# acerbilab/pyvbmc

Measured on AMD Instinct MI355X. Metric: ELBO+entropy evals/sec at D=10, K=50, N=400, Ns=1e6 (1e6-sample-equivalent evals/s), higher is better.
Workload: dtype f64; 1 GPU; BASELINE config 3 per GPU: D=10 K=50 N=400 S=1, Ns=1000000 MC samples per GPU (job Ns=1000000), value+grad _neg_elcbo with soft bounds, eps=philox; parallelism=single GPU

## Files before the change

pyvbmc_amd/_lib.py:

```python
import ctypes as C
import os
import sys
import threading
from pathlib import Path

import numpy as np

_HERE = Path(__file__).resolve().parent
LIB_PATH = Path(os.environ.get("VBMC_HIP_LIB", _HERE / "libvbmc_hip.so"))

EPS_RESIDENT, EPS_PHILOX = 0, 1
MEAN_ZERO, MEAN_CONST, MEAN_NEGQUAD = 0, 1, 2
E_ARG, E_HIP, E_RCCL, E_NODEV, E_UNSUP, E_NONFINITE = -1, -2, -3, -4, -5, -6
W_GP_CHANGED = 1
W_NOT_FUSED = 2


class VbmcHipError(RuntimeError):
    def __init__(self, code, msg):
        super().__init__(f"libvbmc_hip error {code}: {msg}")
        self.code = code


class NoDeviceError(VbmcHipError):
# ... 274 lines not shown
        return bool(b.value), n.value

    def synchronize(self):
        self.check(self._lib.vbmc_synchronize(self._h))

    def set_timing(self, on):
        self.check(self._lib.vbmc_set_timing(self._h, int(on) if on else 0))

    def set_option(self, key, value):
        self.check(self._lib.vbmc_set_option(self._h, key.encode(), int(value)))

    def last_entmc_plan(self):
        out = (C.c_int * 4)()
        self.check(self._lib.vbmc_last_entmc_plan(self._h, out))
        return {"kernel": ("valu", "ws", "small", "mfma", "adam_fused", "ws", "ws")[out[0]] if out[0] >= 0 else None, "rg": out[1],
                "chunks": out[2], "resident_draws": bool(out[3]), "span": out[0] in (5, 6), "adam_tail": out[0] == 6}

    def philox_normals(self, K, n_half, D, seed, row_begin=0, row_count=None):
        row_count = n_half - row_begin if row_count is None else row_count
        out = np.empty((K, row_count, D))
        self.check(self._lib.vbmc_philox_normals(self._h, K, n_half, D, C.c_uint64(seed), row_begin, row_count, ptr(out)))
        return out

    def armed_stats(self):
        out = (C.c_uint64 * 6)()
        self.check(self._lib.vbmc_armed_stats(self._h, out))
        return dict(zip(("hits", "cancels", "late", "ident_checked", "ident_bad", "lost"), (int(v) for v in out)))

    def last_elbo_raw(self, D, K):
        out = np.empty(1 + D * K + 2 * K + D)
        self.check(self._lib.vbmc_last_elbo_raw(self._h, ptr(out), out.size))
# ... 126 lines not shown
```

pyvbmc_amd/csrc/api_elbo.hip:

```cpp
#include <algorithm>
#include <chrono>
#include <cstdlib>
#include <cmath>
#include <cstring>

#include "common.h"
#include "entropy_args.h"

static double soft_bound_loss(const std::vector<double>& x, const double* lb, const double* ub,
                              double tol_con, std::vector<double>* dy) {
  double y = 0.0;
  if (dy) dy->assign(x.size(), 0.0);
  for (size_t i = 0; i < x.size(); ++i) {
    if (x[i] >= lb[i] && x[i] <= ub[i]) continue;
    const double ell = (ub[i] - lb[i]) * tol_con;
    if (x[i] < lb[i]) {
      const double t = (lb[i] - x[i]) / ell;
      y += 0.5 * t * t;
      if (dy) (*dy)[i] = (x[i] - lb[i]) / (ell * ell);
    }
    if (x[i] > ub[i]) {
      const double t = (x[i] - ub[i]) / ell;
      y += 0.5 * t * t;
      if (dy) (*dy)[i] = (x[i] - ub[i]) / (ell * ell);
// ... 208 lines not shown
    if (spin) {
      ctl = ctl_word(ctx, seq_out);
      *(volatile uint64_t*)ctl = 0;
      __builtin_ia32_sfence();
      pa.go = ctl;
      pa.go_seq = seq_out;
      pa.go_timeout = (uint64_t)(ARM_DEVICE_WAIT_MS * 1e5);
      pa.dead = ctx->hd_done + 5;
      plan.a.cancel = ctl;
    }
    HSTAMP(1);
    rc2 = launch_prep(ctx, pa);
    if (rc2) return rc2;
    polled_out = false;
    if (mc) {
      rc2 = entmc_launch_main(ctx, plan);
      if (rc2) return rc2;
      GenSlice ahead_gen;
      DoneSignal done;
      if (can_poll) {
        if (ahead_ok) ahead_gen = entmc_ahead_slice(ctx, plan);
        done.cnt = ctx->d_done_cnt;
        done.sub = ctx->d_done_sub;
        {
          static const int sub_min = [] { const char* e = getenv("VBMC_FIN_SUB_MIN"); return e ? atoi(e) : 256; }();
          done.sub_min = sub_min;
        }
        done.flag = ctx->hd_done;
        done.seq = seq_out;
        done.host_out = raw_out;
        done.host_n = n_raw;
        done.cancel = ctl;
        if (ident) {
          done.ident_src = (const uint64_t*)(ctx->d_done_cnt + 12);
          done.ident_dst = ctx->hd_done + 1;
          done.ident_seed = seed;
        }
        polled_out = true;
        ident_out_flag = ident;
      }
      const GenSlice* gen_here = ahead_gen.n_blocks > 0 ? &ahead_gen : nullptr;
      if (!multi) {
        rc2 = entmc_launch_finish(ctx, plan, polled_out ? stage + n_res : raw_out, gen_here, polled_out ? &done : nullptr);
        if (rc2) return rc2;
      } else {
        rc2 = entmc_launch_finish(ctx, plan, raw_out, nullptr, nullptr);
        if (rc2) return rc2;
        rc2 = comm_allreduce_sum(ctx, raw_out, n_raw);
        if (rc2) return rc2;
        if (polled_out) {
          done.host_out = raw_host;
          rc2 = entmc_launch_publish(ctx, raw_out, done, gen_here);
          if (rc2) return rc2;
        } else {
          HIP_TRY(ctx, hipMemcpyAsync(ctx->h_pinned + n_res, raw_out, sizeof(double) * n_raw,
                                      hipMemcpyDeviceToHost, ctx->stream));
        }
// ... 23 lines not shown
      sp.armed = false;
      const bool force_late = ctx->opt_arm_late_test > 0 && --ctx->opt_arm_late_test == 0;
      if (!force_late && std::chrono::duration<double, std::milli>(clk::now() - sp.t_armed).count() < sp.limit_ms + ARM_LATE_SLACK_MS) {
        ++sp.hits;
        used_armed = true;
        polled = true;
        cur_seq = sp.seq;
        check_ident = sp.ident;
        HSTAMP(1);
      } else {
        *(volatile uint64_t*)ctl_word(ctx, sp.seq) = ~(uint64_t)0;
        __builtin_ia32_sfence();
        HIP_TRY(ctx, stream_wait(ctx));
        HIP_TRY(ctx, hipMemsetAsync(ctx->d_done_cnt, 0, sizeof(int) * 16, ctx->stream));
        HIP_TRY(ctx, hipMemsetAsync(ctx->d_done_sub, 0, sizeof(int) * 16 * 64, ctx->stream));
        ctx->gen_cur = sp.gen_cur_before;
        ctx->ahead.valid = sp.ahead_before_valid;
        ctx->ahead.seed = sp.ahead_before_seed;
        ctx->ahead.buf = sp.ahead_before_buf;
        ctx->ahead.frac = sp.ahead_before_frac;
        ++sp.cancels;
        ++sp.late;
      }
    } else {
      spec_disarm(ctx);
    }
  }
  if (!used_armed) {
    rc = issue(opts->seed, false, polled, cur_seq);
    if (rc) return rc;
// ... 136 lines not shown
    const volatile uint64_t* dead = ctx->h_done + 5;
    unsigned spins = 0;
    for (;;) {
      if (*f == want) break;
      if (*dead == want) return 1;
      __builtin_ia32_pause();
      if ((++spins & 0xFFFF) == 0 && us_since(t_wait) > 5e6) return 2;
    }
    __atomic_thread_fence(__ATOMIC_ACQUIRE);
    return 0;
  };
  auto redo_unarmed = [&](const char* why) -> int {
    HIP_TRY(ctx, stream_wait(ctx));
    HIP_TRY(ctx, hipMemsetAsync(ctx->d_done_cnt, 0, sizeof(int) * 16, ctx->stream));
        HIP_TRY(ctx, hipMemsetAsync(ctx->d_done_sub, 0, sizeof(int) * 16 * 64, ctx->stream));
    ctx->ahead.valid = false;
    if (ctx->ident_retry) return vbmc_fail(ctx, VBMC_E_HIP, "neg_elcbo: %s, twice in a row", why);
    ctx->ident_retry = true;
    const int arm_was = ctx->opt_elbo_arm;
    ctx->opt_elbo_arm = 0;
    const int rc3 = vbmc_neg_elcbo(ctx, theta, n_theta, opts, F, dF, G, H, mu_KxD, sigma_K, lambd_D, w_K, eta_K);
    ctx->opt_elbo_arm = arm_was;
    ctx->ident_retry = false;
    ctx->spec.keep = true;
    return rc3;
  };
  GljHost& o = sc.glj;
  double Gv = 0.0;
  std::vector<double>&dGv = sc.dG, &dHv = sc.dH;
  auto finalize_gp = [&]() -> int {
// ... 136 lines not shown
```

pyvbmc_amd/csrc/common.h:

```cpp
#pragma once
#include <hip/hip_runtime.h>
#include <chrono>

#include <cstdint>
#include <cstdio>
#include <string>
#include <vector>

#include "../../include/vbmc_hip.h"

struct ncclComm;

struct MixLayout {
  int D = 0, K = 0;
  int o_mup = 0;
  int o_mu = 0;
  int o_is2 = 0;
  int o_wc = 0;
  int o_rc = 0;
  int o_lrc = 0;
  int o_sig = 0;
  int o_w = 0;
  int o_lam = 0;
  int o_ilam = 0;
// ... 98 lines not shown
  double* d_epsgen[2] = {nullptr, nullptr};
  size_t d_epsgen_cap[2] = {0, 0};
  int gen_cur = 0;
  struct AheadDraws {
    bool valid = false;
    uint64_t seed = 0;
    int K = 0, D = 0, buf = 0;
    int64_t rows = 0, n_half = 0, row_begin = 0;
    double frac = 1.0;
  } ahead;
  uint64_t* h_done = nullptr;
  uint64_t* hd_done = nullptr;
  int* d_done_cnt = nullptr;
  int* d_done_sub = nullptr;
  uint64_t done_seq = 0;

  double* d_eps = nullptr;
  size_t d_eps_cap = 0;
  int eps_K = 0, eps_D = 0;
  int64_t eps_rows = 0, eps_row_begin = 0, eps_n_half = 0;

  double* d_scratch = nullptr;
  size_t d_scratch_cap = 0;
  double* d_out = nullptr;
  size_t d_out_cap = 0;
  double* d_ptick = nullptr;
  size_t d_ptick_cap = 0;
  double* h_pinned = nullptr;
  double* h_eps = nullptr;
  size_t h_eps_cap = 0;
// ... 13 lines not shown
  int opt_entmc_mfma = 1;
  int opt_elbo_pregen = 1;
  int opt_elbo_ahead = 1;
  int opt_predict_dma = 1;
  int opt_predict_fused = 1;
  int opt_arm_late_test = 0;
  int opt_acq_poll = 1;
  void (*release_cb)(void*) = nullptr;
  void* release_cb_user = nullptr;
  int opt_adam_fused = 1;
  int opt_adam_tail = 1;
  int opt_ident_test = 0;
  bool ident_retry = false;
  int opt_elbo_arm = 1;
  bool counted = false;
  int opt_ws_span = 1;
  int opt_ws_front = 0;
  int opt_ws_pad = -1;
  int opt_mix_bar = 1;
  double* h_pack_dev = nullptr;
  double* h_pack_dev_of = nullptr;
  std::vector<double> exp_eta;
  double exp_eta_sum = 0.0;
  bool exp_eta_valid = false;
  int last_plan[4] = {-1, 0, 0, 0};
  size_t last_raw_off = 0;
  int last_raw_n = 0;

  GpState gp;

// ... 61 lines not shown
                        const double* lambd, const double* w, double* p);
int make_mixture2(vbmc_ctx* ctx, const char* who, int err, int D, int K2, const double* mu2_KxD, const double* sigma2_K,
                  const double* lambd2_D, const double* w2_K, MixLayout& ml2, std::vector<double>& pack2);
int theta_to_arrays(int D, int K, const double* theta, int n_theta, int optimize_mask, double* mu,
                    double* sg, double* lm, double* w, double* eta);
int upload_packed_mixture(vbmc_ctx* ctx);
double* write_pack_to_device(vbmc_ctx* ctx);
int set_mixture_host(vbmc_ctx* ctx, int D, int K, const double* mu_KxD, const double* sigma_K,
                     const double* lambd_D, const double* w_K, const double* eta_K, bool skip_if_same);

int ensure_dev(vbmc_ctx* ctx, double** p, size_t* cap, size_t n_doubles);
int ensure_pinned(vbmc_ctx* ctx, size_t n_doubles);
int randn_with_progress(uint32_t* key, int* pos, int* has_gauss, double* gauss, double* out, int64_t n, int n_threads,
                        void (*progress)(void*, int64_t), void* user);

static inline int raw_len(int D, int K) { return 1 + D * K + 2 * K + D; }

struct DoneSignal {
  int* cnt = nullptr;
  int* sub = nullptr;
  int sub_min = 256;
  uint64_t* flag = nullptr;
  uint64_t seq = 0;
  double* host_out = nullptr;
  int host_n = 0;
  const uint64_t* cancel = nullptr;
  const uint64_t* ident_src = nullptr;
  uint64_t* ident_dst = nullptr;
  uint64_t ident_seed = 0;
  int dev = 0;
// ... 83 lines not shown
  return e;
}
int launch_prep(vbmc_ctx* ctx, const PrepArgs& a);
int launch_prep_on(vbmc_ctx* ctx, hipStream_t stream, const PrepArgs& a);

struct EntPlan;
int entmc_plan(vbmc_ctx* ctx, int64_t ns_per_comp, int eps_mode, uint64_t seed, int64_t row_begin,
               int64_t row_count, int want_grad, EntPlan& p, int gp_items = 0, int gp_per_slot = 0);
bool entmc_take_gp(const vbmc_ctx* ctx, EntPlan& p, const PrepArgs& gp);
void entmc_fill_prep(const vbmc_ctx* ctx, const EntPlan& p, PrepArgs& a);
int entmc_pregen(vbmc_ctx* ctx, EntPlan& p, PrepArgs& a);

int entmc_launch_main(vbmc_ctx* ctx, const EntPlan& p);
int entmc_launch_finish(vbmc_ctx* ctx, const EntPlan& p, double* raw_out, const GenSlice* gen = nullptr,
                        const DoneSignal* done = nullptr);
int entmc_launch_publish(vbmc_ctx* ctx, const double* d_raw, const DoneSignal& done, const GenSlice* gen);
GenSlice entmc_ahead_slice(vbmc_ctx* ctx, const EntPlan& p);
void glj_fill_prep(const vbmc_ctx* ctx, int want_grad, double* res, double* Z, PrepArgs& a);

int launch_entmc(vbmc_ctx* ctx, int64_t ns_per_comp, int eps_mode, uint64_t seed,
                 int64_t row_begin, int64_t row_count, int want_grad, double* d_raw);
int launch_entlb(vbmc_ctx* ctx, double* d_res);
int launch_eps_gen(vbmc_ctx* ctx, hipStream_t st, const GenSlice& g);
int launch_mixture_pdf(vbmc_ctx* ctx, int64_t n, const double* d_x, int log_flag,
                       int grad_flag, double df, double* d_y, double* d_dy);
int launch_mixture_pdf_on(vbmc_ctx* ctx, const double* d_pack, const MixLayout& ml, int64_t n,
                          const double* d_x, int log_flag, double* d_y);
struct Selector {
  int64_t n_exact = 0;
  std::vector<int64_t> cum;
// ... 31 lines not shown
```

pyvbmc_amd/csrc/ctx.hip:

```cpp
#include <cmath>
#include <cstdarg>
#include <cstdlib>
#include <cstring>

#include <sched.h>

#include <cctype>
#include <cstdio>

#include "common.h"

thread_local std::string g_create_err;

int vbmc_fail(vbmc_ctx* ctx, int code, const char* fmt, ...) {
  char buf[1024];
  va_list ap;
  va_start(ap, fmt);
  vsnprintf(buf, sizeof buf, fmt, ap);
  va_end(ap);
  if (ctx)
    ctx->err = buf;
  else
    g_create_err = buf;
  return code;
// ... 29 lines not shown
}

#include <atomic>
static std::atomic<int> g_live_ctx[64];
int vbmc_live_contexts_on(int device) { return device >= 0 && device < 64 ? g_live_ctx[device].load() : 2; }

static void options_from_env(vbmc_ctx* c) {
  const char* e = getenv("VBMC_ENTMC_KERNEL");
  c->opt_entmc_valu = (e && e[0] == 'v') ? 1 : 0;
  e = getenv("VBMC_ELBO_PREGEN");
  c->opt_elbo_pregen = !(e && e[0] == '0');
  e = getenv("VBMC_ELBO_AHEAD");
  c->opt_elbo_ahead = !(e && e[0] == '0');
  e = getenv("VBMC_ELBO_ARM");
  c->opt_elbo_arm = e ? atoi(e) : 1;
  e = getenv("VBMC_ACQ_POLL");
  c->opt_acq_poll = !(e && e[0] == '0');
  e = getenv("VBMC_ADAM_FUSED");
  c->opt_adam_fused = e ? atoi(e) : 1;
  e = getenv("VBMC_RANDN_DEVICE");
  c->opt_randn_dev = e ? (e[0] == '0' ? 0 : e[0] == '2' ? 2 : 1) : 1;
  e = getenv("VBMC_ADAM_TAIL");
  c->opt_adam_tail = e ? atoi(e) : 1;
  e = getenv("VBMC_WS_SPAN");
  c->opt_ws_span = !(e && e[0] == '0');
  e = getenv("VBMC_WS_FRONT");
  if (e) c->opt_ws_front = atoi(e);
  e = getenv("VBMC_WS_PAD");
  if (e) c->opt_ws_pad = atoi(e);
  e = getenv("VBMC_MIX_BAR");
// ... 102 lines not shown
  options_from_env(ctx);
  e = hipSetDevice(device_id);
  if (e == hipSuccess) e = hipGetDeviceProperties(&ctx->prop, device_id);
  if (e == hipSuccess) bind_host_thread(ctx);
  if (e == hipSuccess) e = hipStreamCreateWithFlags(&ctx->stream, hipStreamNonBlocking);
  for (int i = 0; i < 12 && e == hipSuccess; ++i) e = hipEventCreate(&ctx->ev[i]);
  if (e == hipSuccess) e = hipHostMalloc((void**)&ctx->h_done, 64, hipHostMallocDefault);
  if (e == hipSuccess) {
    for (int i = 0; i < 8; ++i) ctx->h_done[i] = 0;
    e = hipHostGetDevicePointer((void**)&ctx->hd_done, ctx->h_done, 0);
  }
  if (e == hipSuccess) e = hipMalloc((void**)&ctx->d_done_cnt, 64);
  if (e == hipSuccess) e = hipMemset(ctx->d_done_cnt, 0, 64);
  if (e == hipSuccess) e = hipMalloc((void**)&ctx->d_done_sub, 16 * 64 * sizeof(int));
  if (e == hipSuccess) e = hipMemset(ctx->d_done_sub, 0, 16 * 64 * sizeof(int));
  if (e != hipSuccess) {
    int rc = vbmc_fail(nullptr, VBMC_E_HIP, "context setup failed: %s", hipGetErrorString(e));
    delete ctx;
    return rc;
  }
  if (strncmp(ctx->prop.gcnArchName, "gfx950", 6) != 0) {
    int rc = vbmc_fail(nullptr, VBMC_E_NODEV, "device %d is %s; this library is built for gfx950 only",
                       device_id, ctx->prop.gcnArchName);
    vbmc_ctx_destroy(ctx);
    return rc;
  }
  if (device_id < 64) g_live_ctx[device_id].fetch_add(1);
  ctx->counted = true;
  *out = ctx;
  return VBMC_OK;
// ... 14 lines not shown
  vbmc_comm_destroy(ctx);
  adam_free(ctx);
  acq_is_free(ctx);
  randn_dev_free(ctx);
  xf_free(ctx);
  double* bufs[] = {ctx->d_mix, ctx->d_mix_fg, ctx->d_acq_fg, ctx->d_stage, ctx->d_eps, ctx->d_scratch, ctx->d_out, ctx->d_ptick, ctx->gp.d_X, ctx->gp.d_XT,
                    ctx->gp.d_alpha, ctx->gp.d_L, ctx->gp.d_Linv, ctx->gp.d_LinvP, ctx->gp.d_sW, ctx->gp.d_hyp,
                    ctx->gp.d_xc, ctx->gp.d_smeta};
  for (double* b : bufs)
    if (b) (void)hipFree(b);
  for (double* b : ctx->d_epsgen)
    if (b) (void)hipFree(b);
  if (ctx->h_done) (void)hipHostFree(ctx->h_done);
  if (ctx->d_done_cnt) (void)hipFree(ctx->d_done_cnt);
  if (ctx->d_done_sub) (void)hipFree(ctx->d_done_sub);
  if (ctx->h_pinned) (void)hipHostFree(ctx->h_pinned);
  if (ctx->h_eps) (void)hipHostFree(ctx->h_eps);
  if (ctx->h_pack) (void)hipHostFree(ctx->h_pack);

  for (hipEvent_t e : ctx->ev)
    if (e) (void)hipEventDestroy(e);
  if (ctx->stream) (void)hipStreamDestroy(ctx->stream);
  delete ctx;
}

const char* vbmc_last_error(const vbmc_ctx* ctx) {
  return ctx ? ctx->err.c_str() : g_create_err.c_str();
}

int vbmc_device_info(const vbmc_ctx* ctx, char* name, int name_len, int* cu_count,
// ... 28 lines not shown
    return VBMC_OK;
  }
  spec_disarm(ctx);
  if (!strcmp(key, "entmc_kernel")) ctx->opt_entmc_valu = value == 1;
  else if (!strcmp(key, "entmc_mfma")) ctx->opt_entmc_mfma = value != 0;
  else if (!strcmp(key, "gp_ship")) ctx->opt_gp_ship = value != 0;
  else if (!strcmp(key, "elbo_pregen")) ctx->opt_elbo_pregen = value != 0;
  else if (!strcmp(key, "elbo_ahead")) ctx->opt_elbo_ahead = value != 0;
  else if (!strcmp(key, "predict_dma")) ctx->opt_predict_dma = value != 0;
  else if (!strcmp(key, "predict_fused")) ctx->opt_predict_fused = value < 0 ? 0 : value > 2 ? 2 : value;
  else if (!strcmp(key, "mix_bar")) ctx->opt_mix_bar = value != 0;
  else if (!strcmp(key, "ws_span")) ctx->opt_ws_span = value != 0;
  else if (!strcmp(key, "ws_pad")) ctx->opt_ws_pad = value > 8 ? 8 : value;
  else if (!strcmp(key, "ws_front")) ctx->opt_ws_front = value < 0 ? 0 : value > 990 ? 990 : value;
  else if (!strcmp(key, "elbo_arm")) ctx->opt_elbo_arm = value < 0 ? 0 : value > 2 ? 2 : value;
  else if (!strcmp(key, "acq_poll")) ctx->opt_acq_poll = value != 0;
  else if (!strcmp(key, "randn_device")) ctx->opt_randn_dev = value < 0 ? 0 : value > 3 ? 3 : value;
  else if (!strcmp(key, "adam_tail")) ctx->opt_adam_tail = value;
  else if (!strcmp(key, "adam_fused")) ctx->opt_adam_fused = value;
  else return vbmc_fail(ctx, VBMC_E_ARG, "vbmc_set_option: unknown key '%s'", key);
  return VBMC_OK;
}

int vbmc_set_gp_watch(vbmc_ctx* ctx, const double* const* ptrs, const int64_t* lens, int n, uint64_t expected) {
  if (!ctx || n < 0 || (n > 0 && (!ptrs || !lens))) return VBMC_E_ARG;
  ctx->gp_watch_ptrs.assign(ptrs, ptrs + n);
  ctx->gp_watch_lens.assign(lens, lens + n);
  ctx->gp_watch_ck = expected;
  return VBMC_OK;
}
// ... 407 lines not shown
```

pyvbmc_amd/csrc/entropy.hip:

```cpp
#include <cstdlib>

#include <algorithm>

#include "common.h"
#include "fastmath.h"
#include "entropy_args.h"
#include "philox.h"
#ifdef FIN_TIMES
__device__ unsigned long long g_glj_stamp;
#define GLJ_STAMP() (g_glj_stamp = wall_clock64())
#endif
#include "glj_block.h"

namespace {

constexpr int WG = 256;
constexpr int WAVES = WG / 64;

__device__ inline double wave_sum(double v) {
  return fm::wave_sum_dpp(v);
}


template <int DP>
// ... 566 lines not shown
  ah.rows = a.row_count;
  ah.n_half = a.n_half;
  ah.row_begin = a.row_begin;
  ah.buf = other;
  ah.frac = frac_end;
  ah.valid = true;
  return make_gen_slice(ctx->d_epsgen[other], K, D, a.row_count, a.n_half, a.row_begin, ah.seed, nullptr, 0.0, frac_end);
}

int entmc_launch_main(vbmc_ctx* ctx, const EntPlan& p) {
  const EntArgs& a = p.a;
  hipEvent_t e0 = ctx->timing ? ctx->ev[0] : nullptr, e1 = ctx->timing ? ctx->ev[1] : nullptr;
  ctx->last_plan[0] = (int)p.kernel;
  ctx->last_plan[1] = a.rg;
  ctx->last_plan[2] = a.chunks;
  ctx->last_plan[3] = a.eps_mode == VBMC_EPS_RESIDENT ? 1 : 0;
  const bool bracket = ctx->timing && (p.kernel == EntKernel::Valu || p.kernel == EntKernel::Small);
  if (bracket) HIP_TRY(ctx, hipEventRecord(ctx->ev[0], ctx->stream));
  switch (p.kernel) {
    case EntKernel::Small: launch_entmc_small(ctx->stream, a, p.DP, p.table); break;
    case EntKernel::Mfma: launch_entmc_mfma(ctx->stream, a, p.DP, p.table, e0, e1); break;
    case EntKernel::Ws:
    case EntKernel::WsSpan:
      switch (p.DP) {
#define VBMC_CASE_WS(dp) case dp: launch_entmc_ws_dp##dp(ctx->stream, a, p.table, e0, e1); break;
        VBMC_WS_DPS(VBMC_CASE_WS)
#undef VBMC_CASE_WS
      }
      break;
    case EntKernel::Valu:
      switch (p.DP) {
// ... 2 lines not shown
#undef VBMC_CASE_VALU
      }
      break;
    default: return vbmc_fail(ctx, VBMC_E_ARG, "entmc: plan names no entropy kernel (%d)", (int)p.kernel);
  }
  if (ctx->timing) {
    if (bracket) HIP_TRY(ctx, hipEventRecord(ctx->ev[1], ctx->stream));
    ctx->ev_valid[0] = true;
  }
  HIP_TRY(ctx, hipGetLastError());
  return 0;
}

namespace {
__global__ __launch_bounds__(256) void eps_gen_kernel(GenSlice g) { gen_slice_block(g, blockIdx.x, threadIdx.x); }
}

GenSlice make_gen_slice(double* eps, int K, int D, int64_t rows, int64_t n_half, int64_t row_begin,
                        uint64_t seed, const int* seed_add, double frac_begin, double frac_end) {
  GenSlice g;
  g.eps = eps;
  g.K = K;
  g.D = D;
  g.rows = rows;
  g.n_half = n_half;
  g.row_begin = row_begin;
  g.seed = seed;
  g.seed_add = seed_add;
  g.nb = (D + 3) / 4;
  auto magic = [](uint64_t d) { return (uint32_t)std::min<uint64_t>(d ? 0x100000000ull / d : 0, 0xFFFFFFFFull); };
// ... 90 lines not shown
```

pyvbmc_amd/csrc/entropy_args.h:

```cpp
#pragma once
#include "common.h"

struct WsSpan {
  int cus = 0;
  int pb = 0;
  int front = 0;
  int nb = 0;
  int pad = 0;
  int R = 0;
  int64_t T = 0;
  __host__ __device__ int nbv() const { return nb + pad; }
  __host__ __device__ int n_parts() const { return cus + pb; }
  __host__ __device__ int64_t W() const { return (int64_t)pb * 1000 + (int64_t)(cus - pb) * front; }
  __host__ __device__ int64_t cw(int u) const {
    return u < 2 * pb ? (int64_t)(u >> 1) * 1000 + (int64_t)(u & 1) * front : (int64_t)pb * 1000 + (int64_t)(u - 2 * pb) * front;
  }
  __host__ __device__ int64_t lo(int u) const { return cw(u) * T / W(); }
  __host__ __device__ int part_of(int64_t g) const {
    const int64_t c = ((g + 1) * W() - 1) / T;
    int u;
    if (c < (int64_t)pb * 1000) {
      const int p = (int)(c / 1000);
      u = 2 * p + ((c - (int64_t)p * 1000) >= front ? 1 : 0);
    } else {
      u = 2 * pb + (int)((c - (int64_t)pb * 1000) / front);
    }
    return u < n_parts() ? u : n_parts() - 1;
  }
  __host__ __device__ int part_of_block(int b) const { return b < cus ? (b < pb ? 2 * b : 2 * pb + (b - pb)) : 2 * (b - cus) + 1; }
};

struct EntArgs {
  const double* mix;
  MixLayout ml;
  const double* eps;
  int64_t eps_rows;
  int64_t n_half;
  int64_t row_begin;
  int64_t row_count;
  uint64_t seed;
  int eps_mode;
  int want_grad;
  double* partial;
  int chunks;
  int stride;
  int rg;
  const void* extra = nullptr;
  int extra_lds = 0;
  int gp_items = 0;
  PrepArgs gp;
  int pair_cus = 0;
  WsSpan sp;
  int gp_wgs = 0;
  const uint64_t* cancel = nullptr;
  const double* ship_src = nullptr;
  double* ship_dst = nullptr;
  int ship_n = 0;
  uint64_t* ship_flag = nullptr;
  uint64_t ship_seq = 0;
};

constexpr int ws_ktmax_for(int K) {
  const int KT = (K + 3) / 4;
  return KT <= 4 ? 4 : KT <= 8 ? 8 : KT <= 10 ? 10 : KT <= 13 ? 13 : KT <= 16 ? 16 : KT <= 20 ? 20 : KT <= 25 ? 25 : 32;
}
constexpr int ws_table_rows(int K) { return 4 * ws_ktmax_for(K); }
constexpr int ws_min_waves(int dp, int ktmax, bool grad) {
#ifdef VBMC_WS_FORCE_WAVES
  return VBMC_WS_FORCE_WAVES;
#else
  return (grad && 4 * dp + 3 * ktmax > 95) ? 1 : 2;
#endif
}

// ... 31 lines not shown
```

pyvbmc_amd/csrc/entropy_mfma.hip:

```cpp
#include <hip/hip_ext.h>

#include <cstdlib>

#include "adam_dev.h"
#include "common.h"
#include "entropy_args.h"
#include "fastmath.h"

namespace {

typedef double double4_t __attribute__((ext_vector_type(4)));
constexpr int WG = 256, WAVES = 4;

__device__ __forceinline__ void exp2_pair(double x1, double x2, double& r1, double& r2) {
  const double t1 = __builtin_rint(x1), t2 = __builtin_rint(x2);
  const double f1 = x1 - t1, f2 = x2 - t2;
  const int n1 = (int)t1, n2 = (int)t2;
  constexpr int EN = VBMC_ENT_EXP2_N;
  constexpr double c[EN] = VBMC_ENT_EXP2_COEFFS;
  double p1 = c[EN - 1], p2 = c[EN - 1];
#pragma unroll
  for (int i = EN - 2; i >= 0; --i) {
    p1 = fma(p1, f1, c[i]);
    p2 = fma(p2, f2, c[i]);
// ... 233 lines not shown
  double* out = a.partial + ((int64_t)j * a.chunks + chunk) * a.stride;
  for (int t = tid; t < a.stride; t += WG) {
    double v = 0.0;
    if (t == 0) {
      for (int wv = 0; wv < WAVES; ++wv) v += sLog[wv];
    } else if (t <= D) {
      for (int wv = 0; wv < WAVES; ++wv) v += sMu[wv * DP + t - 1];
    } else if (t == D + 1) {
      for (int d = 0; d < D; ++d)
        for (int wv = 0; wv < WAVES; ++wv) v += sLam[wv][d];
    } else if (t < 2 * D + 2) {
      for (int wv = 0; wv < WAVES; ++wv) v += sLam[wv][t - (D + 2)];
    } else {
      for (int wv = 0; wv < WAVES; ++wv) v += sWk[wv * KP + t - (2 * D + 2)];
    }
    out[t] = v;
  }
}

template <int DP, int KTILES, int TDP = DP>
void launch_mfma(hipStream_t st, const EntArgs& a, const double* d_table, hipEvent_t e0, hipEvent_t e1) {
  constexpr int TS = DP + 6, KP = 16 * KTILES;
  size_t lds = sizeof(double) * ((size_t)KP * TS + WAVES * DP + WAVES * KP);
  const bool extra_row = a.extra != nullptr;
  if (extra_row && sizeof(double) * (size_t)a.extra_lds > lds) lds = sizeof(double) * (size_t)a.extra_lds;
  auto kern = entmc_mfma_kernel<DP, KTILES, TDP>;
  static size_t lds_limit[64] = {};
  int dev = 0;
  (void)hipGetDevice(&dev);
  if (lds > 32 * 1024 && lds > lds_limit[dev & 63]) {
    (void)hipFuncSetAttribute((const void*)kern, hipFuncAttributeMaxDynamicSharedMemorySize, (int)lds);
    lds_limit[dev & 63] = lds;
// ... 75 lines not shown
```

pyvbmc_amd/csrc/entropy_ws.hip:

```cpp
#include <hip/hip_ext.h>

#include "adam_dev.h"
#include "common.h"
#include "entropy_args.h"
#include "fastmath.h"
#include "glj_block.h"

#ifndef WS_EXP2_N
#define WS_EXP2_N VBMC_ENT_EXP2_N
#endif
constexpr int EN = WS_EXP2_N;
__device__ __forceinline__ double exp2_vc(double x, const double (&c)[EN]) {
  const double t = __builtin_rint(x);
  const double f = x - t;
  const int n = (int)t;
  double p = c[EN - 1];
#pragma unroll
  for (int i = EN - 2; i >= 0; --i) p = fma(p, f, c[i]);
  p = fma(p, f, 1.0);
  return __builtin_amdgcn_ldexp(p, n);
}
__device__ __forceinline__ void exp2_vc2(double x1, double x2, const double (&c)[EN], double& r1,
                                         double& r2) {
  const double t1 = __builtin_rint(x1), t2 = __builtin_rint(x2);
// ... 129 lines not shown
        const int item = m < paired ? 2 * m + (b >= a.pair_cus ? 1 : 0) : paired + m;
        j = item / a.chunks;
        chunk = item - j * a.chunks;
      }
    }
    nb = (int)((a.row_count + 63) >> 6);
    nbv = nb;
    chunk_slot = chunk;
    j_chunk = j;
    const int64_t i0 = (int64_t)chunk * a.rg;
    g_lo = (int64_t)j * nb + (i0 < nb ? i0 : nb);
    g_hi = (int64_t)j * nb + (i0 + a.rg < nb ? i0 + a.rg : nb);
  }
  const int tid = threadIdx.x, lane = tid & 63;
  const int wave = __builtin_amdgcn_readfirstlane(tid >> 6);
  WS_STAMP(0);
  constexpr bool eps_exact = !PHILOX && STAGE != 0;

  double ec[EN];
  {
    int vz;
    asm volatile("v_mov_b32 %0, 0" : "=v"(vz));
#pragma unroll
    for (int i = 0; i < EN; ++i) ec[i] = kExp2C[i + vz];
  }
  WS_STAMP(1);
  bool first_stretch = true;
  for (int64_t g = g_lo; g < g_hi || (first_stretch && !span);) {
  first_stretch = false;
  const int j = span ? (int)(g / nbv) : j_chunk;
// ... 312 lines not shown
    if (t == 0) {
      for (int wv = 0; wv < WAVES; ++wv) v += sRed[wv][0];
    } else if (GRAD) {
      if (t <= D) {
        for (int wv = 0; wv < WAVES; ++wv) v += sRed[wv][t];
      } else if (t == D + 1) {
        for (int d = 0; d < D; ++d)
          for (int wv = 0; wv < WAVES; ++wv) v += sRed[wv][1 + DP + d];
      } else if (t < 2 * D + 2) {
        const int d = t - (D + 2);
        for (int wv = 0; wv < WAVES; ++wv) v += sRed[wv][1 + DP + d];
      } else {
        v = sW[t - (2 * D + 2)];
      }
    }
    out[t] = v;
  }
  if (span) {
    if (ib0 + n_it == nb)
      for (int t = tid; t < (a.chunks - 1 - slot) * a.stride; t += WG) out[a.stride + t] = 0.0;
    __syncthreads();
  }
  g += n_it;
  if (!span) break;
  }
}

template <int DP, int KTMAX>
void launch_one(hipStream_t st, const EntArgs& a_in, const double* d_table, hipEvent_t e0, hipEvent_t e1) {
  EntArgs a = a_in;
  const int K = a.ml.K;
  const int K4 = 4 * KTMAX;
  size_t lds = sizeof(double) * ((size_t)K4 + ws_epi_doubles(DP, KTMAX, a.want_grad != 0));
  const bool philox = a.eps_mode == VBMC_EPS_PHILOX;
  const bool extra_row = a.extra != nullptr && a.want_grad && !philox;
  const dim3 grid = a.sp.cus > 0 ? dim3(a.sp.n_parts() + (a.gp_items > 0 ? a.gp_wgs : 0) + (extra_row ? 1 : 0))
                                 : dim3(a.chunks, K + (extra_row ? 1 : 0) + (a.gp_items > 0 ? 1 : 0));
  const dim3 block(WG);
  if (extra_row && sizeof(double) * (size_t)a.extra_lds > lds) lds = sizeof(double) * (size_t)a.extra_lds;
  if (a.gp_items > 0 && glj_block_lds(a.ml.D, a.gp.N) > lds) lds = glj_block_lds(a.ml.D, a.gp.N);
// ... 53 lines not shown
```

Measured before the change: 12100 evals/s.

## Fuse entropy MC finish reduction into main kernel via last-block tickets

```diff
diff --git a/pyvbmc_amd/_lib.py b/pyvbmc_amd/_lib.py
--- a/pyvbmc_amd/_lib.py
+++ b/pyvbmc_amd/_lib.py
@@ -312,7 +312,8 @@
         out = (C.c_int * 4)()
         self.check(self._lib.vbmc_last_entmc_plan(self._h, out))
         return {"kernel": ("valu", "ws", "small", "mfma", "adam_fused", "ws", "ws")[out[0]] if out[0] >= 0 else None, "rg": out[1],
-                "chunks": out[2], "resident_draws": bool(out[3]), "span": out[0] in (5, 6), "adam_tail": out[0] == 6}
+                "chunks": out[2], "resident_draws": bool(out[3] & 1), "span": out[0] in (5, 6), "adam_tail": out[0] == 6,
+                "fin_in_kernel": bool(out[3] & 2)}
 
     def philox_normals(self, K, n_half, D, seed, row_begin=0, row_count=None):
         row_count = n_half - row_begin if row_count is None else row_count
diff --git a/pyvbmc_amd/csrc/api_elbo.hip b/pyvbmc_amd/csrc/api_elbo.hip
--- a/pyvbmc_amd/csrc/api_elbo.hip
+++ b/pyvbmc_amd/csrc/api_elbo.hip
@@ -246,8 +246,6 @@
     if (rc2) return rc2;
     polled_out = false;
     if (mc) {
-      rc2 = entmc_launch_main(ctx, plan);
-      if (rc2) return rc2;
       GenSlice ahead_gen;
       DoneSignal done;
       if (can_poll) {
@@ -272,7 +270,24 @@
         ident_out_flag = ident;
       }
       const GenSlice* gen_here = ahead_gen.n_blocks > 0 ? &ahead_gen : nullptr;
-      if (!multi) {
+      const bool fin_here = polled_out && !multi && ctx->opt_elbo_fin && ws_form && plan.kernel != EntKernel::Small && ctx->K <= 128 &&
+                            ctx->D <= 32 && (uint64_t)ctx->K * (uint64_t)plan.a.chunks * (uint64_t)plan.a.stride < ((uint64_t)1 << 31);
+      if (fin_here) {
+        EntFin& f = plan.a.fin;
+        f.ticket = ctx->d_fin_tick;
+        f.l1 = ctx->d_fin_l1;
+        f.raw = stage + n_res;
+        f.inv_ns = plan.inv_ns;
+        f.done = done;
+      }
+      rc2 = entmc_launch_main(ctx, plan);
+      if (rc2) return rc2;
+      if (fin_here) {
+        if (gen_here) {
+          rc2 = entmc_launch_tail(ctx, *gen_here, ctl);
+          if (rc2) return rc2;
+        }
+      } else if (!multi) {
         rc2 = entmc_launch_finish(ctx, plan, polled_out ? stage + n_res : raw_out, gen_here, polled_out ? &done : nullptr);
         if (rc2) return rc2;
       } else {
@@ -326,6 +341,7 @@
         HIP_TRY(ctx, stream_wait(ctx));
         HIP_TRY(ctx, hipMemsetAsync(ctx->d_done_cnt, 0, sizeof(int) * 16, ctx->stream));
         HIP_TRY(ctx, hipMemsetAsync(ctx->d_done_sub, 0, sizeof(int) * 16 * 64, ctx->stream));
+        HIP_TRY(ctx, hipMemsetAsync(ctx->d_fin_tick, 0, sizeof(int) * FIN_TICK_WORDS, ctx->stream));
         ctx->gen_cur = sp.gen_cur_before;
         ctx->ahead.valid = sp.ahead_before_valid;
         ctx->ahead.seed = sp.ahead_before_seed;
@@ -492,6 +508,7 @@
     HIP_TRY(ctx, stream_wait(ctx));
     HIP_TRY(ctx, hipMemsetAsync(ctx->d_done_cnt, 0, sizeof(int) * 16, ctx->stream));
         HIP_TRY(ctx, hipMemsetAsync(ctx->d_done_sub, 0, sizeof(int) * 16 * 64, ctx->stream));
+        HIP_TRY(ctx, hipMemsetAsync(ctx->d_fin_tick, 0, sizeof(int) * FIN_TICK_WORDS, ctx->stream));
     ctx->ahead.valid = false;
     if (ctx->ident_retry) return vbmc_fail(ctx, VBMC_E_HIP, "neg_elcbo: %s, twice in a row", why);
     ctx->ident_retry = true;
diff --git a/pyvbmc_amd/csrc/common.h b/pyvbmc_amd/csrc/common.h
--- a/pyvbmc_amd/csrc/common.h
+++ b/pyvbmc_amd/csrc/common.h
@@ -136,6 +136,8 @@
   int* d_done_cnt = nullptr;
   int* d_done_sub = nullptr;
   uint64_t done_seq = 0;
+  int* d_fin_tick = nullptr;
+  double* d_fin_l1 = nullptr;
 
   double* d_eps = nullptr;
   size_t d_eps_cap = 0;
@@ -179,6 +181,7 @@
   bool ident_retry = false;
   int opt_elbo_arm = 1;
   bool counted = false;
+  int opt_elbo_fin = 1;
   int opt_ws_span = 1;
   int opt_ws_front = 0;
   int opt_ws_pad = -1;
@@ -270,6 +273,7 @@
 int randn_with_progress(uint32_t* key, int* pos, int* has_gauss, double* gauss, double* out, int64_t n, int n_threads,
                         void (*progress)(void*, int64_t), void* user);
 
+constexpr int FIN_TICK_WORDS = 128, FIN_L1_STRIDE = 1 + 32 + 128 + 2;
 static inline int raw_len(int D, int K) { return 1 + D * K + 2 * K + D; }
 
 struct DoneSignal {
@@ -383,6 +387,7 @@
 int entmc_launch_main(vbmc_ctx* ctx, const EntPlan& p);
 int entmc_launch_finish(vbmc_ctx* ctx, const EntPlan& p, double* raw_out, const GenSlice* gen = nullptr,
                         const DoneSignal* done = nullptr);
+int entmc_launch_tail(vbmc_ctx* ctx, const GenSlice& gen, const uint64_t* cancel);
 int entmc_launch_publish(vbmc_ctx* ctx, const double* d_raw, const DoneSignal& done, const GenSlice* gen);
 GenSlice entmc_ahead_slice(vbmc_ctx* ctx, const EntPlan& p);
 void glj_fill_prep(const vbmc_ctx* ctx, int want_grad, double* res, double* Z, PrepArgs& a);
diff --git a/pyvbmc_amd/csrc/ctx.hip b/pyvbmc_amd/csrc/ctx.hip
--- a/pyvbmc_amd/csrc/ctx.hip
+++ b/pyvbmc_amd/csrc/ctx.hip
@@ -67,6 +67,8 @@
   c->opt_elbo_ahead = !(e && e[0] == '0');
   e = getenv("VBMC_ELBO_ARM");
   c->opt_elbo_arm = e ? atoi(e) : 1;
+  e = getenv("VBMC_ELBO_FIN");
+  c->opt_elbo_fin = !(e && e[0] == '0');
   e = getenv("VBMC_ACQ_POLL");
   c->opt_acq_poll = !(e && e[0] == '0');
   e = getenv("VBMC_ADAM_FUSED");
@@ -199,6 +201,10 @@
   if (e == hipSuccess) e = hipMemset(ctx->d_done_cnt, 0, 64);
   if (e == hipSuccess) e = hipMalloc((void**)&ctx->d_done_sub, 16 * 64 * sizeof(int));
   if (e == hipSuccess) e = hipMemset(ctx->d_done_sub, 0, 16 * 64 * sizeof(int));
+  if (e == hipSuccess) e = hipMalloc((void**)&ctx->d_fin_tick, FIN_TICK_WORDS * sizeof(int));
+  if (e == hipSuccess) e = hipMemset(ctx->d_fin_tick, 0, FIN_TICK_WORDS * sizeof(int));
+  if (e == hipSuccess) e = hipMalloc((void**)&ctx->d_fin_l1, 64 * FIN_L1_STRIDE * sizeof(double));
+  if (e == hipSuccess) e = hipMemset(ctx->d_fin_l1, 0, 64 * FIN_L1_STRIDE * sizeof(double));
   if (e != hipSuccess) {
     int rc = vbmc_fail(nullptr, VBMC_E_HIP, "context setup failed: %s", hipGetErrorString(e));
     delete ctx;
@@ -243,6 +249,8 @@
   if (ctx->h_done) (void)hipHostFree(ctx->h_done);
   if (ctx->d_done_cnt) (void)hipFree(ctx->d_done_cnt);
   if (ctx->d_done_sub) (void)hipFree(ctx->d_done_sub);
+  if (ctx->d_fin_tick) (void)hipFree(ctx->d_fin_tick);
+  if (ctx->d_fin_l1) (void)hipFree(ctx->d_fin_l1);
   if (ctx->h_pinned) (void)hipHostFree(ctx->h_pinned);
   if (ctx->h_eps) (void)hipHostFree(ctx->h_eps);
   if (ctx->h_pack) (void)hipHostFree(ctx->h_pack);
@@ -301,6 +309,7 @@
   else if (!strcmp(key, "ws_pad")) ctx->opt_ws_pad = value > 8 ? 8 : value;
   else if (!strcmp(key, "ws_front")) ctx->opt_ws_front = value < 0 ? 0 : value > 990 ? 990 : value;
   else if (!strcmp(key, "elbo_arm")) ctx->opt_elbo_arm = value < 0 ? 0 : value > 2 ? 2 : value;
+  else if (!strcmp(key, "elbo_fin")) ctx->opt_elbo_fin = value != 0;
   else if (!strcmp(key, "acq_poll")) ctx->opt_acq_poll = value != 0;
   else if (!strcmp(key, "randn_device")) ctx->opt_randn_dev = value < 0 ? 0 : value > 3 ? 3 : value;
   else if (!strcmp(key, "adam_tail")) ctx->opt_adam_tail = value;
diff --git a/pyvbmc_amd/csrc/entropy.hip b/pyvbmc_amd/csrc/entropy.hip
--- a/pyvbmc_amd/csrc/entropy.hip
+++ b/pyvbmc_amd/csrc/entropy.hip
@@ -604,7 +604,7 @@
   ctx->last_plan[0] = (int)p.kernel;
   ctx->last_plan[1] = a.rg;
   ctx->last_plan[2] = a.chunks;
-  ctx->last_plan[3] = a.eps_mode == VBMC_EPS_RESIDENT ? 1 : 0;
+  ctx->last_plan[3] = (a.eps_mode == VBMC_EPS_RESIDENT ? 1 : 0) | (a.fin.ticket != nullptr ? 2 : 0);
   const bool bracket = ctx->timing && (p.kernel == EntKernel::Valu || p.kernel == EntKernel::Small);
   if (bracket) HIP_TRY(ctx, hipEventRecord(ctx->ev[0], ctx->stream));
   switch (p.kernel) {
@@ -637,6 +637,17 @@
 
 namespace {
 __global__ __launch_bounds__(256) void eps_gen_kernel(GenSlice g) { gen_slice_block(g, blockIdx.x, threadIdx.x); }
+__global__ __launch_bounds__(256) void entmc_tail_kernel(GenSlice g, const uint64_t* cancel) {
+  if (cancel != nullptr && __hip_atomic_load(cancel, __ATOMIC_RELAXED, __HIP_MEMORY_SCOPE_SYSTEM) == ~(uint64_t)0) return;
+  gen_slice_block(g, blockIdx.x, threadIdx.x);
+}
+}
+
+int entmc_launch_tail(vbmc_ctx* ctx, const GenSlice& g, const uint64_t* cancel) {
+  if (g.n_blocks <= 0) return 0;
+  hipLaunchKernelGGL(entmc_tail_kernel, dim3((unsigned)g.n_blocks), dim3(256), 0, ctx->stream, g, cancel);
+  HIP_TRY(ctx, hipGetLastError());
+  return 0;
 }
 
 GenSlice make_gen_slice(double* eps, int K, int D, int64_t rows, int64_t n_half, int64_t row_begin,
diff --git a/pyvbmc_amd/csrc/entropy_args.h b/pyvbmc_amd/csrc/entropy_args.h
--- a/pyvbmc_amd/csrc/entropy_args.h
+++ b/pyvbmc_amd/csrc/entropy_args.h
@@ -30,6 +30,14 @@
   __host__ __device__ int part_of_block(int b) const { return b < cus ? (b < pb ? 2 * b : 2 * pb + (b - pb)) : 2 * (b - cus) + 1; }
 };
 
+struct EntFin {
+  int* ticket = nullptr;
+  double* l1 = nullptr;
+  double* raw = nullptr;
+  double inv_ns = 0.0;
+  DoneSignal done;
+};
+
 struct EntArgs {
   const double* mix;
   MixLayout ml;
@@ -58,6 +66,7 @@
   int ship_n = 0;
   uint64_t* ship_flag = nullptr;
   uint64_t ship_seq = 0;
+  EntFin fin;
 };
 
 constexpr int ws_ktmax_for(int K) {
diff --git a/pyvbmc_amd/csrc/entropy_mfma.hip b/pyvbmc_amd/csrc/entropy_mfma.hip
--- a/pyvbmc_amd/csrc/entropy_mfma.hip
+++ b/pyvbmc_amd/csrc/entropy_mfma.hip
@@ -6,6 +6,7 @@
 #include "common.h"
 #include "entropy_args.h"
 #include "fastmath.h"
+#include "fin_inkernel.h"
 
 namespace {
 
@@ -271,8 +272,10 @@
     } else {
       for (int wv = 0; wv < WAVES; ++wv) v += sWk[wv * KP + t - (2 * D + 2)];
     }
-    out[t] = v;
-  }
+    if (a.fin.ticket != nullptr) __hip_atomic_store(out + t, v, __ATOMIC_RELAXED, __HIP_MEMORY_SCOPE_AGENT);
+    else out[t] = v;
+  }
+  if (a.fin.ticket != nullptr) fin_ik::run<1>((fin_ik::kernarg)__builtin_amdgcn_kernarg_segment_ptr(), dyn, j);
 }
 
 template <int DP, int KTILES, int TDP = DP>
diff --git a/pyvbmc_amd/csrc/entropy_ws.hip b/pyvbmc_amd/csrc/entropy_ws.hip
--- a/pyvbmc_amd/csrc/entropy_ws.hip
+++ b/pyvbmc_amd/csrc/entropy_ws.hip
@@ -4,6 +4,7 @@
 #include "common.h"
 #include "entropy_args.h"
 #include "fastmath.h"
+#include "fin_inkernel.h"
 #include "glj_block.h"
 
 #ifndef WS_EXP2_N
@@ -167,6 +168,7 @@
   }
   const int tid = threadIdx.x, lane = tid & 63;
   const int wave = __builtin_amdgcn_readfirstlane(tid >> 6);
+  const bool fin_here = a.fin.ticket != nullptr;
   WS_STAMP(0);
   constexpr bool eps_exact = !PHILOX && STAGE != 0;
 
@@ -509,16 +511,21 @@
         v = sW[t - (2 * D + 2)];
       }
     }
-    out[t] = v;
+    if (fin_here) __hip_atomic_store(out + t, v, __ATOMIC_RELAXED, __HIP_MEMORY_SCOPE_AGENT);
+    else out[t] = v;
   }
   if (span) {
     if (ib0 + n_it == nb)
-      for (int t = tid; t < (a.chunks - 1 - slot) * a.stride; t += WG) out[a.stride + t] = 0.0;
+      for (int t = tid; t < (a.chunks - 1 - slot) * a.stride; t += WG) {
+        if (fin_here) __hip_atomic_store(out + a.stride + t, 0.0, __ATOMIC_RELAXED, __HIP_MEMORY_SCOPE_AGENT);
+        else out[a.stride + t] = 0.0;
+      }
     __syncthreads();
   }
   g += n_it;
   if (!span) break;
   }
+  if (fin_here) fin_ik::run<ws_min_waves(DP, KTMAX, GRAD)>((fin_ik::kernarg)__builtin_amdgcn_kernarg_segment_ptr(), dyn, span ? part : j_chunk);
 }
 
 template <int DP, int KTMAX>
diff --git a/pyvbmc_amd/csrc/fin_inkernel.h b/pyvbmc_amd/csrc/fin_inkernel.h
--- /dev/null
+++ b/pyvbmc_amd/csrc/fin_inkernel.h
@@ -0,0 +1,217 @@
+#pragma once
+#include "common.h"
+#include "entropy_args.h"
+#include "fastmath.h"
+
+namespace fin_ik {
+
+using gcd = const __attribute__((address_space(1))) double*;
+using gd = __attribute__((address_space(1))) double*;
+using gi = __attribute__((address_space(1))) int*;
+using gu64 = __attribute__((address_space(1))) uint64_t*;
+using kernarg = const __attribute__((address_space(4))) char*;
+
+__device__ __forceinline__ double ld(const double* p) { return __hip_atomic_load((gcd)p, __ATOMIC_RELAXED, __HIP_MEMORY_SCOPE_AGENT); }
+__device__ __forceinline__ void st(double* p, double v) { __hip_atomic_store((gd)p, v, __ATOMIC_RELAXED, __HIP_MEMORY_SCOPE_AGENT); }
+__device__ __forceinline__ void drain() { __builtin_amdgcn_s_waitcnt(0x0F70); }
+
+__device__ __forceinline__ bool arrive_last(int* word, int target, int* s_word) {
+  if (threadIdx.x == 0) {
+    int last = 0;
+    if (__hip_atomic_fetch_add((gi)word, 1, __ATOMIC_RELAXED, __HIP_MEMORY_SCOPE_AGENT) == target - 1) {
+      __hip_atomic_store((gi)word, 0, __ATOMIC_RELAXED, __HIP_MEMORY_SCOPE_AGENT);
+      last = 1;
+    }
+    *s_word = last;
+  }
+  __syncthreads();
+  const bool last = *s_word != 0;
+  __syncthreads();
+  return last;
+}
+
+constexpr int FOLD_U = 12;
+constexpr int L1_PAD = 2;
+
+__device__ __forceinline__ void level1(const EntArgs& a, int g) {
+  const int D = a.ml.D, K = a.ml.K, chunks = a.chunks, stride = a.stride;
+  const int tid = threadIdx.x, lane = tid & 63, wave = tid >> 6;
+  const double* w = a.mix + a.ml.o_w;
+  const double* sig = a.mix + a.ml.o_sig;
+  const double* ilam = a.mix + a.ml.o_ilam;
+  const double* mup = a.mix + a.ml.o_mup;
+  const double* is2 = a.mix + a.ml.o_is2;
+  const double* partial = a.partial;
+  const double inv_ns = a.fin.inv_ns;
+  const unsigned jstride = (unsigned)(chunks * stride);
+  double* l1row = a.fin.l1 + (size_t)g * (1 + D + K + L1_PAD);
+  const int ncol = a.want_grad ? 1 + D + K : 1;
+  if (tid < ncol) {
+    const int col = tid;
+    const bool is_lam = col >= 1 && col <= D;
+    const unsigned off = col == 0 ? 0u : is_lam ? (unsigned)(2 + D + (col - 1)) : (unsigned)(2 + 2 * D + (col - 1 - D));
+    double acc = 0.0;
+    for (int r0 = 0; r0 < K; r0 += 64) {
+      const int r = r0 + g;
+      const int rc = min(r, K - 1);
+      const double c = r < K ? (is_lam ? w[rc] * sig[rc] : w[rc]) : 0.0;
+      const unsigned b = (unsigned)rc * jstride + off;
+      for (int c0 = 0; c0 < chunks; c0 += FOLD_U) {
+        double x[FOLD_U];
+#pragma unroll
+        for (int u = 0; u < FOLD_U; ++u) x[u] = ld(partial + (b + (unsigned)(min(c0 + u, chunks - 1) * stride)));
+#pragma unroll
+        for (int u = 0; u < FOLD_U; ++u)
+          if (c0 + u < chunks) acc = col == 0 ? acc - c * x[u] : acc + c * x[u];
+      }
+    }
+    st(l1row + col, acc);
+  }
+  if (!a.want_grad) return;
+  constexpr int NI = 9;
+  for (int jj = g; jj < K; jj += 64) {
+    double v[NI];
+#pragma unroll
+    for (int i = 0; i < NI; ++i) v[i] = 0.0;
+    for (int c = lane; c < chunks; c += 64) {
+      const double* row = partial + ((int64_t)jj * chunks + c) * stride;
+#pragma unroll
+      for (int i = 0; i < NI; ++i) {
+        const int idx = wave + 4 * i;
+        if (idx < D + 2) v[i] += ld(row + (idx <= D ? 1 + idx : 0));
+      }
+    }
+    for (int r0 = 0; r0 < K; r0 += 64) {
+      const int r = r0 + lane;
+      const int rc = min(r, K - 1);
+      const double wis = w[rc] * is2[rc];
+      double cf[NI];
+#pragma unroll
+      for (int i = 0; i < NI; ++i) {
+        const int d = wave + 4 * i;
+        cf[i] = (r < K && d < D) ? wis * (mup[jj * D + d] - mup[rc * D + d]) : 0.0;
+      }
+      const unsigned b = (unsigned)jj * jstride + (unsigned)(2 + 2 * D + rc);
+      for (int c0 = 0; c0 < chunks; c0 += FOLD_U) {
+        double x[FOLD_U];
+#pragma unroll
+        for (int u = 0; u < FOLD_U; ++u) x[u] = ld(partial + (b + (unsigned)(min(c0 + u, chunks - 1) * stride)));
+#pragma unroll
+        for (int u = 0; u < FOLD_U; ++u)
+          if (c0 + u < chunks) {
+#pragma unroll
+            for (int i = 0; i < NI; ++i)
+              if (wave + 4 * i < D) v[i] = fma(cf[i], x[u], v[i]);
+          }
+      }
+    }
+#pragma unroll
+    for (int i = 0; i < NI; ++i) {
+      const int idx = wave + 4 * i;
+      if (idx >= D + 2) continue;
+      const double s = fm::wave_sum_dpp(v[i]);
+      if (lane != 0) continue;
+      if (idx < D) st(a.fin.raw + 1 + jj * D + idx, s * w[jj] * inv_ns * ilam[idx]);
+      else if (idx == D) st(a.fin.raw + 1 + D * K + jj, s * w[jj] * inv_ns);
+      else st(l1row + 1 + D + K + (jj >> 6), s);
+    }
+  }
+}
+
+__device__ __forceinline__ void level2(const EntArgs& a) {
+  const int D = a.ml.D, K = a.ml.K;
+  const int tid = threadIdx.x, lane = tid & 63, wave = tid >> 6;
+  const int n_groups = K < 64 ? K : 64;
+  const int L1S = 1 + D + K + L1_PAD;
+  const double* ilam = a.mix + a.ml.o_ilam;
+  const double inv_ns = a.fin.inv_ns;
+  double* raw = a.fin.raw;
+  const double* l1 = a.fin.l1;
+  const int ncol = a.want_grad ? 1 + D + K : 1;
+  constexpr int U = 4;
+  const double* mine = l1 + (size_t)min(lane, n_groups - 1) * L1S;
+  for (int base = 0; base < ncol; base += 4 * U) {
+    double x[U], sl[U];
+#pragma unroll
+    for (int u = 0; u < U; ++u) {
+      const int col = min(base + 4 * u + wave, ncol - 1);
+      const double xv = ld(mine + col);
+      x[u] = lane < n_groups ? xv : 0.0;
+      const int uu = col > D ? col - 1 - D : 0;
+      sl[u] = ld(l1 + (size_t)(uu & 63) * L1S + 1 + D + K + (uu >> 6));
+    }
+#pragma unroll
+    for (int u = 0; u < U; ++u) {
+      const int col = base + 4 * u + wave;
+      const double s = fm::wave_sum_dpp(x[u]);
+      if (col >= ncol || lane != 0) continue;
+      if (col == 0) st(raw, s * inv_ns);
+      else if (col <= D) st(raw + 1 + D * K + K + (col - 1), s * inv_ns * ilam[col - 1]);
+      else st(raw + 1 + D * K + K + D + (col - 1 - D), -inv_ns * (sl[u] + s));
+    }
+  }
+  const int n = 1 + D * K + 2 * K + D;
+  if (!a.want_grad)
+    for (int t = 1 + tid; t < n; t += 256) st(raw + t, 0.0);
+  drain();
+  __syncthreads();
+  const DoneSignal& done = a.fin.done;
+  if (done.ident_dst && tid == 255) {
+    __hip_atomic_store((gu64)done.ident_dst, *done.ident_src, __ATOMIC_RELAXED, __HIP_MEMORY_SCOPE_SYSTEM);
+    __hip_atomic_store((gu64)done.ident_dst + 1, done.ident_seed, __ATOMIC_RELAXED, __HIP_MEMORY_SCOPE_SYSTEM);
+  }
+  for (int base = 0; base < done.host_n; base += 256 * 8) {
+    double v[8];
+#pragma unroll
+    for (int u = 0; u < 8; ++u) v[u] = ld(raw + min(base + u * 256 + tid, done.host_n - 1));
+#pragma unroll
+    for (int u = 0; u < 8; ++u)
+      __hip_atomic_store((gd)done.host_out + min(base + u * 256 + tid, done.host_n - 1), v[u], __ATOMIC_RELAXED, __HIP_MEMORY_SCOPE_SYSTEM);
+  }
+  drain();
+  __syncthreads();
+  if (tid == 0) __hip_atomic_store((gu64)done.flag, done.seq, __ATOMIC_RELAXED, __HIP_MEMORY_SCOPE_SYSTEM);
+}
+
+template <int MIN_WAVES>
+static __device__ __noinline__ __attribute__((not_tail_called)) void run(kernarg ka, double* lds, int where) {
+  EntArgs a;
+  __builtin_memcpy(&a, (const char*)ka, sizeof(EntArgs));
+  const int K = a.ml.K;
+  int* s_word = (int*)lds;
+  drain();
+  __syncthreads();
+  const bool span = a.sp.cus > 0;
+  int j_lo = where, j_hi = where, nbv = 0, nb = 0;
+  int64_t g_lo = 0, g_hi = 0;
+  if (span) {
+    g_lo = a.sp.lo(where);
+    g_hi = a.sp.lo(where + 1);
+    if (g_hi <= g_lo) return;
+    nbv = a.sp.nbv();
+    nb = a.sp.nb;
+    j_lo = (int)(g_lo / nbv);
+    j_hi = (int)((g_hi - 1) / nbv);
+  }
+  for (int j = j_lo; j <= j_hi; ++j) {
+    if (span) {
+      const int64_t c0 = (int64_t)j * nbv, c1 = c0 + nb;
+      const int64_t s0 = g_lo > c0 ? g_lo : c0, s1 = g_hi < c1 ? g_hi : c1;
+      if (s0 >= s1) continue;
+    }
+    const int g = j & 63;
+    int target = 0;
+    if (threadIdx.x == 0)
+      for (int jj = g; jj < K; jj += 64)
+        target += span ? a.sp.part_of((int64_t)jj * nbv + nb - 1) - a.sp.part_of((int64_t)jj * nbv) + 1 : a.chunks;
+    if (!arrive_last(a.fin.ticket + g, target, s_word)) continue;
+    level1(a, g);
+    drain();
+    __syncthreads();
+    if (!arrive_last(a.fin.ticket + 64, K < 64 ? K : 64, s_word)) continue;
+    level2(a);
+    return;
+  }
+}
+
+}
```

New measurement: 10420 evals/s. -13.8%, worse.
